# SGI-2022/Latent-Diffusion-Models-for-Shape-SDFs

Measured on AMD Instinct MI355X. Metric: SDF queries/sec on 256^3 grid (+ DDPM sample steps/sec), higher is better.
Workload: dtype bf16; 1 GPU; config4: decode B=64 shapes on a 256^3 grid on 1 rank (the whole grid is the one slab: no gather); batch=64, grid=256, latent_dim=256, decoder=DeepSDF 8x512 skip@4, parallelism=zslab1

## Files before the change

latent-diffusion-models-for-shape-sdfs_amd/csrc/decoder_fs.hip:

```cpp
#include "decoder_common.h"

namespace ldm {
namespace {
using namespace dec;

constexpr int kFsD = 4;

constexpr int kFsStep = 2048;
constexpr int kFsAct = 33 * 4 * 1024;
constexpr int kFsRed = 4 * 4 * 64 * 4;
constexpr int kFsWl = 512 * 4;
#ifndef FS_STAMP
#define FS_STAMP 0
#endif
constexpr int kFsStamp = FS_STAMP ? 128 * 8 : 0;
#ifndef FS_ABL
#define FS_ABL 0
#endif
static_assert(FS_ABL == 0 || FS_STAMP, "ablations are diagnostic builds");
constexpr int kFsLds = kFsAct + kFsRed + kFsWl + kFsStamp;
static_assert(kFsLds <= 160 * 1024, "LDS");

__host__ __device__ constexpr int fs_nparts(int S) { return S == 256 ? 15 : 16; }
__host__ __device__ constexpr int fs_nsteps(int S) { return S == 256 ? 384 : 448; }

template <typename T>
__global__ void fs_aux_pack_kernel(const float* __restrict__ beta, const float* __restrict__ wxyz,
                                   int B, T* __restrict__ aux) {
    const int id = blockIdx.x * blockDim.x + threadIdx.x;
    if (id >= B * 4 * 4 * 2 * 64) return;
    const int lane = id & 63;
    const int i = (id >> 6) & 1;
    const int slot = (id >> 7) & 3;
    const int w = (id >> 9) & 3;
    const int b = id >> 11;
    const int li = slot >> 1;
    const int p = slot & 1;
    float v[8] = {0, 0, 0, 0, 0, 0, 0, 0};
    if (lane < 32) {
        const int f = 128 * w + 64 * p + 32 * i + lane;
        const float* wx = wxyz + ((size_t)li * kHidden + f) * 3;
        const float bb = beta[((size_t)b * 2 + li) * kHidden + f];
        const float hi = Elem<T>::round(bb);
        v[0] = wx[0]; v[1] = wx[1]; v[2] = wx[2];
        v[3] = wx[0]; v[4] = wx[1]; v[5] = wx[2];
        v[6] = hi;    v[7] = bb - hi;
    }
    T* o = aux + (size_t)id * 8;
#pragma unroll
    for (int e = 0; e < 8; ++e) o[e] = (T)v[e];
}

struct FArgs {
    const uint8_t* stream;
    const uint8_t* aux;
    const float* w_last;
    const float* xyz;
    float* out;
    float b_last;
    int npts, tiles_per_shape, n_tiles;
    int N, k0;
    float vs, origin;
    const int32_t* bricks;
    const int32_t* count;
    int nb, nbt;
    GridDiv gd;
};

enum FsEpi { FE_NONE = 0, FE_LATE = 1, FE_EARLY = 2, FE_FIN0 = 3, FE_FIN1 = 4 };

struct FSrc {
    bool shape;
    uint32_t off;
    bool none = false;
};

struct FCtx {
    int lane, wave, h;
    uint32_t voff;
    char* smem;
    __amdgpu_buffer_rsrc_t rw;
    __amdgpu_buffer_rsrc_t ra;
    uint32_t s_beg, s_end;
    uint32_t s_iss;
    uint32_t baux_w;
    uint32_t aux_w;
    uint32_t aux_next;
    u32x4 auxn[2];
    u32x4 ring[kFsD][2];
    u32x4 b[4];
    float part[4];
    float* out;
    int npts, prev_shape, prev_local;
    float b_last;
    unsigned long long* st;
    int st_i;
    bool st_on;
    const int32_t* bricks;
    int N, nb, nbt;
};

__device__ __forceinline__ void stamp(FCtx& c) {
    if (FS_STAMP) {
        if (c.st_on && c.lane == 0 && c.st_i < 128) c.st[c.st_i] = __builtin_readcyclecounter();
        ++c.st_i;
    }
}

__device__ __forceinline__ u32x4 bld(__amdgpu_buffer_rsrc_t r, uint32_t voff, uint32_t soff) {
    return __builtin_bit_cast(u32x4, __builtin_amdgcn_raw_buffer_load_b128(r, voff, soff, 0));
}

__device__ __forceinline__ void load_aux(FCtx& c, FSrc s) {
    if (s.none) return;
    const __amdgpu_buffer_rsrc_t r = s.shape ? c.ra : c.rw;
    c.auxn[0] = bld(r, c.voff, s.off);
    c.auxn[1] = bld(r, c.voff + 1024u, s.off);
}

__device__ __forceinline__ uint32_t opaque(uint32_t v) {
    asm volatile("" : "+v"(v));
    return v;
}

__device__ __forceinline__ int opaque_s(int v) {
    asm volatile("" : "+s"(v));
    return v;
}

__device__ __forceinline__ char* lds_at(const FCtx& c, uint32_t off) {
    return c.smem + (opaque(c.voff) + off);
}
__device__ __forceinline__ u32x4* act_w(const FCtx& c, int late) {
    return reinterpret_cast<u32x4*>(lds_at(c, (uint32_t)(late + 4 * c.wave) * 4096u));
}
__device__ __forceinline__ const f32x4* wl_at(const FCtx& c, int p, int i) {
    const uint32_t h = opaque(c.voff) >> 9;
    return reinterpret_cast<const f32x4*>(
        c.smem + kFsAct + kFsRed + (((c.wave * 2 + p) * 2 + i) * 2) * 64 + h * 64);
}

__device__ __forceinline__ float* red_w(const FCtx& c) {
    return reinterpret_cast<float*>(c.smem + kFsAct + c.wave * 4 * 64 * 4 + (opaque(c.voff) >> 2));
}

__device__ __forceinline__ void fs_bar() {
    if (FS_ABL & 4) return;
    asm volatile("s_waitcnt lgkmcnt(0)\n\ts_barrier" ::: "memory");
}

__device__ __forceinline__ void read_b(FCtx& c, int pos) {
    const u32x4* p = reinterpret_cast<const u32x4*>(lds_at(c, pos * 4096));
#pragma unroll
    for (int n = 0; n < 4; ++n) c.b[n] = p[n * 64];
}

__device__ __forceinline__ void issue(FCtx& c, int r) {
    const uint32_t so = c.s_iss + (uint32_t)(r >> 1) * 2u * kFsStep;
    const uint32_t vo = c.voff + (uint32_t)(r & 1) * kFsStep;
    if (FS_ABL & 1) return;
    c.ring[r][0] = bld(c.rw, vo, so);
    c.ring[r][1] = bld(c.rw, vo + 1024u, so);
}

__device__ __forceinline__ void next_group(FCtx& c) {
    c.s_iss += 4u * kFsStep;
    if (c.s_iss == c.s_end) c.s_iss = c.s_beg;
}

__device__ __forceinline__ float relu_f(float x) {
    return __builtin_bit_cast(float, max(__builtin_bit_cast(int, x), 0));
}

__device__ __forceinline__ float acc_read(float a) {
    asm volatile("" : "+a"(a));
    return a;
}

template <typename T, int EK>
__device__ __forceinline__ void epi_unit(FCtx& c, const f32x16 (&accY)[2][4], int u) {
    const int t = u >> 1, s = u & 1;
    const int i = t >> 2, n = t & 3;
    if (FS_ABL & 2) return;
    if (EK == FE_LATE || EK == FE_EARLY) {
        u32x4 f;
#pragma unroll
        for (int q = 0; q < 4; ++q)
            f[q] = relu2(Elem<T>::pack(accY[i][n][8 * s + 2 * q], accY[i][n][8 * s + 2 * q + 1]));
        u32x4* p = act_w(c, EK == FE_LATE ? 16 : 0);
        p[((2 * i + s) * 4 + n) * 64] = f;
    } else if (EK == FE_FIN0 || EK == FE_FIN1) {
        const f32x4* w = wl_at(c, EK == FE_FIN0 ? 0 : 1, i);
        float part = c.part[n];
#pragma unroll
        for (int q = 2 * s; q < 2 * s + 2; ++q) {
            const f32x4 wv = w[q];
#pragma unroll
            for (int e = 0; e < 4; ++e) {
                const float v = EK == FE_FIN1 ? acc_read(accY[i][n][4 * q + e])
                                              : accY[i][n][4 * q + e];
                part = fmaf(relu_f(v), wv[e], part);
            }
        }
        c.part[n] = part;
    }
}

template <typename T, int EK>
__device__ __forceinline__ void epi_step(FCtx& c, const f32x16 (&accY)[2][4], int k) {
    if (EK == FE_NONE || k == 15) return;
    epi_unit<T, EK>(c, accY, k);
    if (k == 14) epi_unit<T, EK>(c, accY, 15);
    if (EK == FE_FIN1 && k == 14) {
        float* rw = red_w(c);
#pragma unroll
        for (int n = 0; n < 4; ++n) {
            rw[n * 64] = c.part[n];
            c.part[n] = 0.f;
        }
    }
}

__device__ __forceinline__ void fin_store(const FCtx& c, int shape, int local) {
    const int lane = (int)(opaque(c.voff) >> 4);
    if (local < 0 || lane >= 32) return;
    const float* rr = reinterpret_cast<const float*>(
        c.smem + kFsAct + c.wave * 64 * 4 + (opaque(c.voff) >> 2));
    float s = 0.f;
#pragma unroll
    for (int w = 0; w < 4; ++w) s += rr[w * 4 * 64] + rr[w * 4 * 64 + 32];
    const int pt = local * kTilePoints + 32 * c.wave + lane;
    if (pt < c.npts) {
        const __amdgpu_buffer_rsrc_t ro = __builtin_amdgcn_make_buffer_rsrc(
            (void*)(c.out + (size_t)shape * c.npts), (short)0, 0x7ffffff0, 0x00020000);
        __builtin_amdgcn_raw_buffer_store_b32(__builtin_bit_cast(uint32_t, tanhf(s + c.b_last)),
                                              ro, (uint32_t)pt * 4u, 0, 2 );
    }
}

__device__ __forceinline__ int list_at(const int32_t* list, int i) {
    typedef const __attribute__((address_space(4))) int32_t* const_i32;
    return ((const_i32)(uintptr_t)list)[i];
}

__device__ __forceinline__ void brick_origin(int gid, int nb_, int& shape, int& i0, int& j0,
                                             int& k0) {
    const int nb = opaque_s(nb_);
    const int nb2 = nb * nb, nb3 = nb2 * nb;
    shape = gid / nb3;
    const int id = gid - shape * nb3;
    const int bz = id / nb2, r = id - bz * nb2;
    const int by = r / nb;
    i0 = 8 * (r - by * nb);
    j0 = 8 * by;
    k0 = 8 * bz;
}

__device__ __forceinline__ void fin_store_bricks(const FCtx& c, int tile) {
    const int lane = (int)(opaque(c.voff) >> 4);
    if (tile < 0 || lane >= 32) return;
    const float* rr = reinterpret_cast<const float*>(
        c.smem + kFsAct + c.wave * 64 * 4 + (opaque(c.voff) >> 2));
    float s = 0.f;
#pragma unroll
    for (int w = 0; w < 4; ++w) s += rr[w * 4 * 64] + rr[w * 4 * 64 + 32];
    const int gid = list_at(c.bricks, tile >> 2);
    LDM_DASSERT(gid >= 0 && gid < c.nbt);
    int shape, i0, j0, k0;
    brick_origin(gid, c.nb, shape, i0, j0, k0);
    const int idx = 128 * (tile & 3) + 32 * c.wave + lane;
    const int i = i0 + (idx & 7), j = j0 + ((idx >> 3) & 7);
    const int k = k0 + 2 * (tile & 3) + (c.wave >> 1);
    const int N = c.N;
    if ((unsigned)gid < (unsigned)c.nbt && i < N && j < N && k < N) {
        const __amdgpu_buffer_rsrc_t ro = __builtin_amdgcn_make_buffer_rsrc(
            (void*)(c.out + ((size_t)shape * N + k) * N * N), (short)0, 0x7ffffff0, 0x00020000);
        __builtin_amdgcn_raw_buffer_store_b32(__builtin_bit_cast(uint32_t, tanhf(s + c.b_last)),
                                              ro, (uint32_t)(j * N + i) * 4u, 0, 2 );
    }
}

template <int MODE>
__device__ __forceinline__ void fin_store_mode(const FCtx& c) {
    if (MODE == kModeBricks) fin_store_bricks(c, c.prev_local);
    else fin_store(c, c.prev_shape, c.prev_local);
}

__device__ __forceinline__ void valu_slot(int v) {
    if (v == 2) __builtin_amdgcn_sched_group_barrier(0x002, 2, 0);
    else if (v == 4) __builtin_amdgcn_sched_group_barrier(0x002, 4, 0);
}

template <typename T>
__device__ __forceinline__ void mfma_pair(f32x16 (&acc)[2][4], const u32x4& a0, const u32x4& a1,
                                          const u32x4& b, int n) {
    acc[0][n] = Elem<T>::mfma(a0, b, acc[0][n]);
    acc[1][n] = Elem<T>::mfma(a1, b, acc[1][n]);
}

template <typename T, int EK, int K0, int BAR>
__device__ __forceinline__ void group4(FCtx& c, f32x16 (&acc)[2][4], const f32x16 (&accY)[2][4],
                                       int p0) {
    constexpr int BP = 1;
    const char* gbase = lds_at(c, (p0 + 1) * 4096);
#pragma unroll
    for (int r = 0; r < 4; ++r) {
        const u32x4* nb = reinterpret_cast<const u32x4*>(gbase + r * 4096);
        const u32x4 a0 = c.ring[r][0], a1 = c.ring[r][1];
        const int k = K0 + r;
        const int V = (EK == FE_NONE || k == 15) ? 0 : (k == 14 ? 4 : 2);
        if (r == BAR) {
#pragma unroll
            for (int n = 0; n < BP; ++n) mfma_pair<T>(acc, a0, a1, c.b[n], n);
            for (int n = 0; n < BP; ++n) {
                __builtin_amdgcn_sched_group_barrier(0x008, 2, 0);
            }
            __builtin_amdgcn_sched_barrier(0);
            fs_bar();
            __builtin_amdgcn_sched_barrier(0);
#pragma unroll
            for (int n = 0; n < BP; ++n) c.b[n] = nb[n * 64];
#pragma unroll
            for (int n = BP; n < 4; ++n) {
                mfma_pair<T>(acc, a0, a1, c.b[n], n);
                c.b[n] = nb[n * 64];
            }
            issue(c, r);
            epi_step<T, EK>(c, accY, k);
            for (int n = 0; n < BP; ++n) __builtin_amdgcn_sched_group_barrier(0x100, 1, 0);
            for (int n = BP; n < 4; ++n) {
                __builtin_amdgcn_sched_group_barrier(0x008, 1, 0);
                valu_slot(V);
                __builtin_amdgcn_sched_group_barrier(0x008, 1, 0);
                __builtin_amdgcn_sched_group_barrier(0x100, 1, 0);
                valu_slot(V);
            }
        } else {
#pragma unroll
            for (int n = 0; n < 4; ++n) {
                mfma_pair<T>(acc, a0, a1, c.b[n], n);
                c.b[n] = nb[n * 64];
            }
            issue(c, r);
            epi_step<T, EK>(c, accY, k);
#pragma unroll
            for (int n = 0; n < 4; ++n) {
                __builtin_amdgcn_sched_group_barrier(0x008, 1, 0);
                valu_slot(V);
                __builtin_amdgcn_sched_group_barrier(0x008, 1, 0);
                __builtin_amdgcn_sched_group_barrier(0x100, 1, 0);
                valu_slot(V);
            }
        }
        __builtin_amdgcn_sched_group_barrier(0x020, 2, 0);
        __builtin_amdgcn_sched_barrier(0);
    }
    next_group(c);
}

template <typename T, int EK, bool BAR>
__device__ __forceinline__ void steps16e(FCtx& c, f32x16 (&acc)[2][4],
                                         const f32x16 (&accY)[2][4], int p0) {
    group4<T, EK, 0, -1>(c, acc, accY, p0);
    group4<T, EK, 4, -1>(c, acc, accY, p0 + 4);
    group4<T, EK, 8, -1>(c, acc, accY, p0 + 8);
    group4<T, EK, 12, BAR ? 3 : -1>(c, acc, accY, p0 + 12);
}

template <typename T>
__device__ __forceinline__ void steps_plain(FCtx& c, f32x16 (&acc)[2][4],
                                            const f32x16 (&accY)[2][4], int pos0, int j0, int j1) {
#pragma unroll 1
    for (int j = j0; j < j1; j += 4) group4<T, FE_NONE, 0, -1>(c, acc, accY, pos0 + j);
}

template <typename T, int EK, bool E16, int MODE = kModeGrid>
__device__ __forceinline__ void run_part(FCtx& c, f32x16 (&acc)[2][4], const f32x16 (&accY)[2][4],
                                         int nk, bool mid, bool endbar, FSrc naux, int pos0,
                                         bool bar0) {
    const f32x16 zero = {};
    const u32x4 a0 = c.auxn[0], a1 = c.auxn[1];
    if (bar0) {
#pragma unroll
        for (int n = 0; n < 4; ++n) {
            acc[0][n] = Elem<T>::mfma(a0, c.b[n], zero);
            acc[1][n] = Elem<T>::mfma(a1, c.b[n], zero);
        }
        load_aux(c, naux);
        fs_bar();
        read_b(c, pos0);
    } else {
        const u32x4* p = reinterpret_cast<const u32x4*>(lds_at(c, pos0 * 4096));
#pragma unroll
        for (int n = 0; n < 4; ++n) {
            acc[0][n] = Elem<T>::mfma(a0, c.b[n], zero);
            acc[1][n] = Elem<T>::mfma(a1, c.b[n], zero);
            c.b[n] = p[n * 64];
        }
        load_aux(c, naux);
#pragma unroll
        for (int n = 0; n < 4; ++n) {
            __builtin_amdgcn_sched_group_barrier(0x008, 2, 0);
            __builtin_amdgcn_sched_group_barrier(0x100, 1, 0);
        }
        __builtin_amdgcn_sched_group_barrier(0x020, 2, 0);
        __builtin_amdgcn_sched_barrier(0);
    }
    stamp(c);
    if (!E16 && EK != FE_NONE) {
        if (mid || (endbar && nk == 16)) steps16e<T, EK, true>(c, acc, accY, pos0);
        else steps16e<T, EK, false>(c, acc, accY, pos0);
        if (EK == FE_FIN1) {
            stamp(c);
            fin_store_mode<MODE>(c);
        }
        stamp(c);
        if (endbar && nk == 32) {
            steps_plain<T>(c, acc, accY, pos0, 16, 28);
            group4<T, FE_NONE, 0, 3>(c, acc, accY, pos0 + 28);
        } else {
            steps_plain<T>(c, acc, accY, pos0, 16, nk);
        }
    } else if (E16) {
        steps_plain<T>(c, acc, accY, pos0, 0, 12);
        group4<T, FE_NONE, 0, 3>(c, acc, accY, pos0 + 12);
        stamp(c);
        if (endbar) steps16e<T, EK, true>(c, acc, accY, pos0 + 16);
        else steps16e<T, EK, false>(c, acc, accY, pos0 + 16);
    } else {
        steps_plain<T>(c, acc, accY, pos0, 0, nk < 16 ? nk : 16);
        stamp(c);
        steps_plain<T>(c, acc, accY, pos0, 16, nk);
    }
    stamp(c);
}

template <typename T>
__device__ __forceinline__ void acc_to_lds(FCtx& c, const f32x16 (&acc)[2][4]) {
    u32x4* p = act_w(c, 16);
#pragma unroll
    for (int i = 0; i < 2; ++i)
#pragma unroll
        for (int n = 0; n < 4; ++n) {
            u32x4 f0, f1;
            acc_to_frags<T>(acc[i][n], f0, f1);
            p[(2 * i * 4 + n) * 64] = f0;
            p[((2 * i + 1) * 4 + n) * 64] = f1;
        }
}

template <typename T, bool LATE>
__device__ __forceinline__ void layer0_part(FCtx& c, FSrc naux) {
    const u32x4 a[2] = {c.auxn[0], c.auxn[1]};
    u32x4* p = act_w(c, LATE ? 16 : 0);
    f32x16 t[2];
    t[0] = Elem<T>::mfma_v(a[0], c.b[0]);
#pragma unroll
    for (int q = 0; q < 8; ++q) {
        const int i = q & 1, n = q >> 1;
        if (q < 7) t[(q + 1) & 1] = Elem<T>::mfma_v(a[(q + 1) & 1], c.b[(q + 1) >> 1]);
        if (q == 0) {
            asm volatile("s_nop 10" : "+v"(t[0]));
            load_aux(c, naux);
            stamp(c);
        }
        __builtin_amdgcn_sched_barrier(0);
        u32x4 f0, f1;
        acc_to_frags<T>(t[q & 1], f0, f1);
        p[(2 * i * 4 + n) * 64] = f0;
        p[((2 * i + 1) * 4 + n) * 64] = f1;
        __builtin_amdgcn_sched_barrier(0);
    }
    stamp(c);
}

template <typename T, int S, int MODE>
__global__ __launch_bounds__(256, 1) void dec_fs_kernel(FArgs a) {
    __shared__ __attribute__((aligned(16))) char smem[kFsLds];
    FCtx c;
    c.lane = threadIdx.x & 63;
    c.wave = __builtin_amdgcn_readfirstlane(threadIdx.x >> 6);
    c.h = c.lane >> 5;
    c.voff = (uint32_t)c.lane * 16u;
    c.smem = smem;
    c.out = a.out;
    c.npts = a.npts;
    c.b_last = a.b_last;
    c.prev_shape = 0;
    c.prev_local = -1;
    c.st = reinterpret_cast<unsigned long long*>(smem + kFsAct + kFsRed + kFsWl);
    c.st_i = 0;
    c.st_on = false;
    float* wl = reinterpret_cast<float*>(smem + kFsAct + kFsRed);

    for (int i = threadIdx.x; i < 512; i += 256) wl[i] = a.w_last[i];
    __syncthreads();
    const int n_tiles = MODE == kModeBricks ? 4 * min(max(a.count[0], 0), a.nbt) : a.n_tiles;
    if (MODE == kModeBricks) {
        c.bricks = a.bricks;
        c.N = a.N;
        c.nb = a.nb;
        c.nbt = a.nbt;
    }
    if ((int)blockIdx.x >= n_tiles) return;

    constexpr int NST = fs_nsteps(S);
    constexpr int NP = fs_nparts(S);
    constexpr uint32_t kFlags = 0x00020000u;
    c.rw = __builtin_amdgcn_make_buffer_rsrc((void*)a.stream, (short)0, 0x7ffffff0, kFlags);
    c.ra = __builtin_amdgcn_make_buffer_rsrc((void*)a.aux, (short)0, 0x7ffffff0, kFlags);
    c.s_beg = (uint32_t)c.wave * NST * kFsStep;
    c.s_end = c.s_beg + NST * kFsStep;
    c.s_iss = c.s_beg;
    c.baux_w = (uint32_t)(4 * NST + c.wave * NP) * kFsStep;
    auto brick_of = [&](int tile) -> int {
        return min(max(list_at(a.bricks, tile >> 2), 0), a.nbt - 1);
    };
    auto shape_aux = [&](int tile) -> uint32_t {
        if (MODE == kModeBricks) {
            const int nb = opaque_s(a.nb);
            return ((uint32_t)(brick_of(tile) / (nb * nb * nb)) * 4u + (uint32_t)c.wave) * 4u *
                   kFsStep;
        }
        return ((uint32_t)(tile / a.tiles_per_shape) * 4u + (uint32_t)c.wave) * 4u * kFsStep;
    };
    auto bias = [&](int pi) -> FSrc { return FSrc{false, c.baux_w + (uint32_t)pi * kFsStep}; };
    auto shp = [&](int slot) -> FSrc { return FSrc{true, c.aux_w + (uint32_t)slot * kFsStep}; };
    c.aux_w = shape_aux(blockIdx.x);
#pragma unroll
    for (int r = 0; r < kFsD; ++r) issue(c, r);
    next_group(c);

    f32x16 accA[2][4], accB[2][4];
#pragma unroll
    for (int i = 0; i < 2; ++i)
#pragma unroll
        for (int n = 0; n < 4; ++n) accB[i][n] = f32x16{};
#pragma unroll
    for (int n = 0; n < 4; ++n) c.part[n] = 0.f;
#pragma unroll 1
    for (int tile = blockIdx.x; tile < n_tiles; tile += gridDim.x) {
        int shape, local, bi0 = 0, bj0 = 0, bk0 = 0;
        if (MODE == kModeBricks) {
            brick_origin(brick_of(tile), a.nb, shape, bi0, bj0, bk0);
            local = tile;
        } else {
            shape = tile / a.tiles_per_shape;
            local = tile - shape * a.tiles_per_shape;
        }
        {
            const int nt = tile + (int)gridDim.x;
            c.aux_next = nt < n_tiles ? shape_aux(nt) : c.aux_w;
        }
        c.st_on = FS_STAMP && c.wave == 0 && tile == (int)blockIdx.x + (int)gridDim.x;
        c.st_i = 0;
        stamp(c);
        load_aux(c, shp(0));
        const uint32_t lv = opaque(c.voff);
        const bool hi = lv >= 512u;
        const uint32_t p0 = (uint32_t)local * kTilePoints;
        uint32_t ti = 0, tj = 0, tk = 0;
        if (MODE == kModeGrid) {
            grid_first(p0, (uint32_t)a.N, a.gd, ti, tj, tk);
            tk += (uint32_t)a.k0;
        }
        const float* row = nullptr;
        if (MODE == kModePoints) {
            row = a.xyz + (size_t)shape * a.npts * 3;
            asm volatile("" : "+s"(row));
        }
#pragma unroll
        for (int n = 0; n < 4; ++n) {
            int pt = local * kTilePoints + 32 * n + (int)((lv >> 4) & 31u);
            if (pt >= a.npts) pt = a.npts - 1;
            float x, y, z;
            if (MODE == kModeBricks) {
                const int idx = 128 * (tile & 3) + 32 * n + (int)((lv >> 4) & 31u);
                const int m = a.N - 1;
                x = grid_axis(min(bi0 + (idx & 7), m), a.vs, a.origin);
                y = grid_axis(min(bj0 + ((idx >> 3) & 7), m), a.vs, a.origin);
                z = grid_axis(min(bk0 + (idx >> 6), m), a.vs, a.origin);
            } else if (MODE == kModePoints) {
                const float* qq = row + (size_t)pt * 3;
                x = qq[0];
                y = qq[1];
                z = qq[2];
            } else {
                const uint32_t off =
                    grid_tail_off(p0, 32u * n + ((lv >> 4) & 31u), (uint32_t)a.npts);
                uint32_t vi, vj, vk;
                grid_voxel(ti, tj, tk, off, (uint32_t)a.N, a.gd.m, vi, vj, vk);
                x = grid_axis((int)vi, a.vs, a.origin);
                y = grid_axis((int)vj, a.vs, a.origin);
                z = grid_axis((int)vk, a.vs, a.origin);
            }
            const float xh = Elem<T>::round(x), yh = Elem<T>::round(y), zh = Elem<T>::round(z);
            u32x4 f;
            f[0] = hi ? 0u : Elem<T>::pack(xh, yh);
            f[1] = hi ? 0u : Elem<T>::pack(zh, x - xh);
            f[2] = hi ? 0u : Elem<T>::pack(y - yh, z - zh);
            f[3] = hi ? 0u : Elem<T>::pack(1.f, 1.f);
            reinterpret_cast<u32x4*>(lds_at(c, 32u * 4096u))[n * 64] = f;
        }
        read_b(c, 32);

        layer0_part<T, false>(c, shp(1));
        layer0_part<T, true>(c, bias(2));

        int pi = 2;
        run_part<T, FE_FIN1, false, MODE>(c, accA, accB, 32, true, false, bias(pi + 1), 0, true);
        run_part<T, FE_EARLY, true>(c, accB, accA, 32, true, true, bias(pi + 2), 0, false);
        pi += 2;
        constexpr int L2P = S == 256 ? 3 : 4;
#pragma unroll 1
        for (int l = 2; l < L2P; ++l, pi += 2) {
            const FSrc nx = (S == 512 && l == 3) ? shp(2) : bias(pi + 2);
            run_part<T, FE_LATE, false>(c, accA, accB, 32, true, false, bias(pi + 1), 0, false);
            run_part<T, FE_EARLY, true>(c, accB, accA, 32, true, true, nx, 0, false);
        }
        if (S == 256) {
            run_part<T, FE_LATE, false>(c, accA, accB, 32, true, false, shp(2), 0, false);
            fs_bar();
            acc_to_lds<T>(c, accA);
            stamp(c);
            run_part<T, FE_NONE, false>(c, accA, accB, 16, false, false, shp(3), 16, true);
            run_part<T, FE_EARLY, false>(c, accB, accA, 16, false, true, bias(pi + 3), 16,
                                             false);
            pi += 3;
        } else {
            run_part<T, FE_LATE, false>(c, accA, accB, 32, true, false, shp(3), 0, false);
            run_part<T, FE_EARLY, true>(c, accB, accA, 32, true, true, bias(pi + 2), 0, false);
            pi += 2;
        }
#pragma unroll 1
        for (int l = 5; l < 7; ++l, pi += 2) {
            run_part<T, FE_LATE, false>(c, accA, accB, 32, true, false, bias(pi + 1), 0, false);
            run_part<T, FE_EARLY, true>(c, accB, accA, 32, true, true, bias(pi + 2), 0, false);
        }
        run_part<T, FE_LATE, false>(c, accA, accB, 32, true, false, bias(pi + 1), 0, false);
        run_part<T, FE_FIN0, false>(c, accB, accA, 32, false, true, FSrc{true, 0, true}, 0,
                                        false);
        c.prev_shape = shape;
        c.prev_local = local;
        c.aux_w = c.aux_next;
    }
#pragma unroll
    for (int u = 0; u < 16; ++u) epi_unit<T, FE_FIN1>(c, accB, u);
    {
        float* rw = red_w(c);
#pragma unroll
        for (int n = 0; n < 4; ++n) rw[n * 64] = c.part[n];
    }
    fs_bar();
    fin_store_mode<MODE>(c);
    asm volatile("s_waitcnt vmcnt(0)" ::: "memory");
    if (FS_STAMP && c.wave == 0) {
        __builtin_amdgcn_s_waitcnt(0);
        for (int k = c.lane; k < 128; k += 64)
            reinterpret_cast<unsigned long long*>(a.out)[(size_t)blockIdx.x * 128 + k] = c.st[k];
    }
}

template <typename T, int S>
void launch_fs(const FArgs& a, bool points, hipStream_t s, int grid) {
    if (points)
        hipLaunchKernelGGL((dec_fs_kernel<T, S, kModePoints>), dim3(grid), dim3(256), 0, s, a);
    else
        hipLaunchKernelGGL((dec_fs_kernel<T, S, kModeGrid>), dim3(grid), dim3(256), 0, s, a);
}

template <typename T, int S>
void launch_fs_bricks(const FArgs& a, hipStream_t s, int grid) {
    hipLaunchKernelGGL((dec_fs_kernel<T, S, kModeBricks>), dim3(grid), dim3(256), 0, s, a);
}

}

size_t decoder_fs_aux_bytes(int B) { return (size_t)B * 4 * 4 * kFsStep; }

int decoder_fs_n_stages(int skip_width) { return fs_nsteps(skip_width == 253 ? 256 : 512); }

int decoder_fs_fwd(const ldm_decoder_t* w, const float* beta, const float* xyz, int B, int npts,
                   int N, int k0, float vs, float origin, float* out, void* ws, size_t ws_bytes,
                   hipStream_t s, int num_cus, const int32_t* bricks, const int32_t* count,
                   int n_bricks) {
    const int S = w->skip_width == 253 ? 256 : 512;
    LDM_REQUIRE(w->n_stages == fs_nsteps(S), LDM_EINVAL, "split layout: n_stages %d != %d",
                w->n_stages, fs_nsteps(S));
    LDM_REQUIRE(ws != nullptr && ws_bytes >= decoder_fs_aux_bytes(B) && LDM_ALIGNED(ws, 16),
                LDM_ENOSPC, "workspace too small: need %zu bytes, got %zu",
                decoder_fs_aux_bytes(B), ws_bytes);
    LDM_REQUIRE((size_t)B * 4 * 4 * kFsStep < 0x7ffffff0u, LDM_EINVAL,
                "split layout: %d shapes exceed the aux buffer range", B);
    {
        const int n = B * 4 * 4 * 2 * 64;
        if (w->dtype == LDM_BF16)
            hipLaunchKernelGGL(fs_aux_pack_kernel<__bf16>, dim3((n + 255) / 256), dim3(256), 0, s,
                               beta, w->wxyz, B, (__bf16*)ws);
        else
            hipLaunchKernelGGL(fs_aux_pack_kernel<_Float16>, dim3((n + 255) / 256), dim3(256), 0,
                               s, beta, w->wxyz, B, (_Float16*)ws);
        if (int e = launch_status("fs_aux_pack")) return e;
    }
    FArgs a;
    a.stream = (const uint8_t*)w->weights;
    a.aux = (const uint8_t*)ws;
    a.w_last = w->w_last;
    a.xyz = xyz;
    a.out = out;
    a.b_last = w->b_last;
    a.npts = npts;
    a.tiles_per_shape = (npts + kTilePoints - 1) / kTilePoints;
    a.n_tiles = B * a.tiles_per_shape;
    a.bricks = bricks;
    a.count = count;
    a.nb = (N + 7) / 8;
    a.nbt = n_bricks;
    const int mode = bricks ? kModeBricks : xyz ? kModePoints : kModeGrid;
    if (mode == kModeBricks) a.n_tiles = 4 * n_bricks;
    a.N = N;
    a.k0 = k0;
    a.vs = vs;
    a.origin = origin;
    a.gd = mode == kModeGrid ? grid_div(N) : GridDiv{0, 0, 0};
    const int grid = a.n_tiles < num_cus ? a.n_tiles : num_cus;
    if (mode != kModeBricks) {
        const bool points = mode == kModePoints;
        if (w->dtype == LDM_BF16) {
            if (S == 256) launch_fs<__bf16, 256>(a, points, s, grid);
            else launch_fs<__bf16, 512>(a, points, s, grid);
        } else {
            if (S == 256) launch_fs<_Float16, 256>(a, points, s, grid);
            else launch_fs<_Float16, 512>(a, points, s, grid);
        }
    } else if (w->dtype == LDM_BF16) {
        if (S == 256) launch_fs_bricks<__bf16, 256>(a, s, grid);
        else launch_fs_bricks<__bf16, 512>(a, s, grid);
    } else {
        if (S == 256) launch_fs_bricks<_Float16, 256>(a, s, grid);
        else launch_fs_bricks<_Float16, 512>(a, s, grid);
    }
    return launch_status("ldm_decoder_fwd(split)");
}

}
```

Measured before the change: 475.2 million queries/s.

## Pin epilogue accumulator reads in AGPRs and split E16 conversion into convert/write phases

Adds a PIN flag so most epilogues read accumulators through an AGPR asm constraint. This keeps the compiler from copying whole accumulator tiles into VGPRs early. For S=256 the E16 path now converts half of the layer's accumulators into a 16-entry register buffer while MFMAs run, then writes them to LDS in a separate group. The other layers keep the original late/early epilogue interleave. The aim is lower register pressure and better overlap of the epilogue with MFMA, at the cost of extra live registers (ef[16]) and a more intricate schedule.

```diff
diff --git a/latent-diffusion-models-for-shape-sdfs_amd/csrc/decoder_fs.hip b/latent-diffusion-models-for-shape-sdfs_amd/csrc/decoder_fs.hip
--- a/latent-diffusion-models-for-shape-sdfs_amd/csrc/decoder_fs.hip
+++ b/latent-diffusion-models-for-shape-sdfs_amd/csrc/decoder_fs.hip
@@ -67,7 +67,8 @@
     GridDiv gd;
 };
 
-enum FsEpi { FE_NONE = 0, FE_LATE = 1, FE_EARLY = 2, FE_FIN0 = 3, FE_FIN1 = 4 };
+enum FsEpi { FE_NONE = 0, FE_LATE = 1, FE_EARLY = 2, FE_FIN0 = 3, FE_FIN1 = 4, FE_CVT = 5,
+             FE_WR = 6, FE_PIN = 8 };
 
 struct FSrc {
     bool shape;
@@ -90,6 +91,7 @@
     u32x4 ring[kFsD][2];
     u32x4 b[4];
     float part[4];
+    u32x4 ef[16];
     float* out;
     int npts, prev_shape, prev_local;
     float b_last;
@@ -177,18 +179,22 @@
     return a;
 }
 
-template <typename T, int EK>
-__device__ __forceinline__ void epi_unit(FCtx& c, const f32x16 (&accY)[2][4], int u) {
+template <typename T, int EKP>
+__device__ __forceinline__ void epi_unit(FCtx& c, const f32x16 (&accY)[2][4], int u,
+                                         u32x4* wbase) {
+    constexpr int EK = EKP & 7;
+    constexpr bool PIN = (EKP & FE_PIN) != 0 || EK == FE_FIN1;
     const int t = u >> 1, s = u & 1;
     const int i = t >> 2, n = t & 3;
     if (FS_ABL & 2) return;
     if (EK == FE_LATE || EK == FE_EARLY) {
         u32x4 f;
 #pragma unroll
-        for (int q = 0; q < 4; ++q)
-            f[q] = relu2(Elem<T>::pack(accY[i][n][8 * s + 2 * q], accY[i][n][8 * s + 2 * q + 1]));
-        u32x4* p = act_w(c, EK == FE_LATE ? 16 : 0);
-        p[((2 * i + s) * 4 + n) * 64] = f;
+        for (int q = 0; q < 4; ++q) {
+            const float lo = accY[i][n][8 * s + 2 * q], hi = accY[i][n][8 * s + 2 * q + 1];
+            f[q] = relu2(PIN ? Elem<T>::pack(acc_read(lo), acc_read(hi)) : Elem<T>::pack(lo, hi));
+        }
+        wbase[((2 * i + s) * 4 + n) * 64] = f;
     } else if (EK == FE_FIN0 || EK == FE_FIN1) {
         const f32x4* w = wl_at(c, EK == FE_FIN0 ? 0 : 1, i);
         float part = c.part[n];
@@ -197,8 +203,7 @@
             const f32x4 wv = w[q];
 #pragma unroll
             for (int e = 0; e < 4; ++e) {
-                const float v = EK == FE_FIN1 ? acc_read(accY[i][n][4 * q + e])
-                                              : accY[i][n][4 * q + e];
+                const float v = PIN ? acc_read(accY[i][n][4 * q + e]) : accY[i][n][4 * q + e];
                 part = fmaf(relu_f(v), wv[e], part);
             }
         }
@@ -206,11 +211,40 @@
     }
 }
 
-template <typename T, int EK>
-__device__ __forceinline__ void epi_step(FCtx& c, const f32x16 (&accY)[2][4], int k) {
+template <typename T, int EKP>
+__device__ __forceinline__ void epi_step(FCtx& c, const f32x16 (&accY)[2][4], int k,
+                                         u32x4* wbase) {
+    constexpr int EK = EKP & 7;
     if (EK == FE_NONE || k == 15) return;
-    epi_unit<T, EK>(c, accY, k);
-    if (k == 14) epi_unit<T, EK>(c, accY, 15);
+    if (EK == FE_CVT) {
+        if ((FS_ABL & 2) || k >= 8) return;
+        u32x4 f0, f1;
+#pragma unroll
+        for (int q = 0; q < 4; ++q) {
+            const f32x16& a = accY[k >> 2][k & 3];
+            f0[q] = relu2(Elem<T>::pack(acc_read(a[2 * q]), acc_read(a[2 * q + 1])));
+            f1[q] = relu2(Elem<T>::pack(acc_read(a[8 + 2 * q]), acc_read(a[8 + 2 * q + 1])));
+        }
+        c.ef[2 * k] = f0;
+        c.ef[2 * k + 1] = f1;
+        return;
+    }
+    if (EK == FE_WR) {
+        if ((FS_ABL & 2) || k >= 4) return;
+#pragma unroll
+        for (int t = 2 * k; t < 2 * k + 2; ++t) {
+            const int i = t >> 2, n = t & 3;
+            wbase[(2 * i * 4 + n) * 64] = c.ef[2 * t];
+            wbase[((2 * i + 1) * 4 + n) * 64] = c.ef[2 * t + 1];
+        }
+        return;
+    }
+    epi_unit<T, EKP>(c, accY, k, wbase);
+    if (k == 14) epi_unit<T, EKP>(c, accY, 15, wbase);
+    if (EK == FE_FIN0 && k == 14) {
+#pragma unroll
+        for (int n = 0; n < 4; ++n) asm volatile("" : "+v"(c.part[n]));
+    }
     if (EK == FE_FIN1 && k == 14) {
         float* rw = red_w(c);
 #pragma unroll
@@ -298,17 +332,22 @@
     acc[1][n] = Elem<T>::mfma(a1, b, acc[1][n]);
 }
 
-template <typename T, int EK, int K0, int BAR>
+template <typename T, int EKP, int K0, int BAR>
 __device__ __forceinline__ void group4(FCtx& c, f32x16 (&acc)[2][4], const f32x16 (&accY)[2][4],
                                        int p0) {
+    constexpr int EK = EKP & 7;
     constexpr int BP = 1;
+    u32x4* wbase = nullptr;
+    if (EK == FE_LATE) wbase = act_w(c, 16);
+    if (EK == FE_EARLY || EK == FE_WR) wbase = act_w(c, 0);
     const char* gbase = lds_at(c, (p0 + 1) * 4096);
 #pragma unroll
     for (int r = 0; r < 4; ++r) {
         const u32x4* nb = reinterpret_cast<const u32x4*>(gbase + r * 4096);
         const u32x4 a0 = c.ring[r][0], a1 = c.ring[r][1];
         const int k = K0 + r;
-        const int V = (EK == FE_NONE || k == 15) ? 0 : (k == 14 ? 4 : 2);
+        const int V = (EK == FE_NONE || EK == FE_WR || k == 15) ? 0
+                      : (k == 14 || EK == FE_CVT) ? 4 : 2;
         if (r == BAR) {
 #pragma unroll
             for (int n = 0; n < BP; ++n) mfma_pair<T>(acc, a0, a1, c.b[n], n);
@@ -326,7 +365,7 @@
                 c.b[n] = nb[n * 64];
             }
             issue(c, r);
-            epi_step<T, EK>(c, accY, k);
+            epi_step<T, EKP>(c, accY, k, wbase);
             for (int n = 0; n < BP; ++n) __builtin_amdgcn_sched_group_barrier(0x100, 1, 0);
             for (int n = BP; n < 4; ++n) {
                 __builtin_amdgcn_sched_group_barrier(0x008, 1, 0);
@@ -342,7 +381,7 @@
                 c.b[n] = nb[n * 64];
             }
             issue(c, r);
-            epi_step<T, EK>(c, accY, k);
+            epi_step<T, EKP>(c, accY, k, wbase);
 #pragma unroll
             for (int n = 0; n < 4; ++n) {
                 __builtin_amdgcn_sched_group_barrier(0x008, 1, 0);
@@ -374,10 +413,11 @@
     for (int j = j0; j < j1; j += 4) group4<T, FE_NONE, 0, -1>(c, acc, accY, pos0 + j);
 }
 
-template <typename T, int EK, bool E16, int MODE = kModeGrid>
+template <typename T, int EKP, bool E16, int MODE = kModeGrid>
 __device__ __forceinline__ void run_part(FCtx& c, f32x16 (&acc)[2][4], const f32x16 (&accY)[2][4],
                                          int nk, bool mid, bool endbar, FSrc naux, int pos0,
                                          bool bar0) {
+    constexpr int EK = EKP & 7;
     const f32x16 zero = {};
     const u32x4 a0 = c.auxn[0], a1 = c.auxn[1];
     if (bar0) {
@@ -406,10 +446,16 @@
         __builtin_amdgcn_sched_group_barrier(0x020, 2, 0);
         __builtin_amdgcn_sched_barrier(0);
     }
+    if (EK == FE_NONE) {
+#pragma unroll
+        for (int i = 0; i < 2; ++i)
+#pragma unroll
+            for (int n = 0; n < 4; ++n) asm volatile("" ::"a"(accY[i][n]));
+    }
     stamp(c);
     if (!E16 && EK != FE_NONE) {
-        if (mid || (endbar && nk == 16)) steps16e<T, EK, true>(c, acc, accY, pos0);
-        else steps16e<T, EK, false>(c, acc, accY, pos0);
+        if (mid || (endbar && nk == 16)) steps16e<T, EKP, true>(c, acc, accY, pos0);
+        else steps16e<T, EKP, false>(c, acc, accY, pos0);
         if (EK == FE_FIN1) {
             stamp(c);
             fin_store_mode<MODE>(c);
@@ -421,12 +467,21 @@
         } else {
             steps_plain<T>(c, acc, accY, pos0, 16, nk);
         }
-    } else if (E16) {
+    } else if (E16 && (EKP & FE_PIN)) {
         steps_plain<T>(c, acc, accY, pos0, 0, 12);
         group4<T, FE_NONE, 0, 3>(c, acc, accY, pos0 + 12);
         stamp(c);
-        if (endbar) steps16e<T, EK, true>(c, acc, accY, pos0 + 16);
-        else steps16e<T, EK, false>(c, acc, accY, pos0 + 16);
+        if (endbar) steps16e<T, EKP, true>(c, acc, accY, pos0 + 16);
+        else steps16e<T, EKP, false>(c, acc, accY, pos0 + 16);
+    } else if (E16) {
+        static_assert(!E16 || EK == FE_EARLY, "E16 parts convert part 0 of their own layer");
+        steps_plain<T>(c, acc, accY, pos0, 0, 8);
+        group4<T, FE_CVT, 0, -1>(c, acc, accY, pos0 + 8);
+        group4<T, FE_CVT, 4, 3>(c, acc, accY, pos0 + 12);
+        stamp(c);
+        group4<T, FE_WR, 0, -1>(c, acc, accY, pos0 + 16);
+        steps_plain<T>(c, acc, accY, pos0, 20, 28);
+        group4<T, FE_NONE, 0, 3>(c, acc, accY, pos0 + 28);
     } else {
         steps_plain<T>(c, acc, accY, pos0, 0, nk < 16 ? nk : 16);
         stamp(c);
@@ -607,6 +662,7 @@
         layer0_part<T, false>(c, shp(1));
         layer0_part<T, true>(c, bias(2));
 
+        constexpr int kPinW = S == 512 ? FE_PIN : 0;
         int pi = 2;
         run_part<T, FE_FIN1, false, MODE>(c, accA, accB, 32, true, false, bias(pi + 1), 0, true);
         run_part<T, FE_EARLY, true>(c, accB, accA, 32, true, true, bias(pi + 2), 0, false);
@@ -615,37 +671,44 @@
 #pragma unroll 1
         for (int l = 2; l < L2P; ++l, pi += 2) {
             const FSrc nx = (S == 512 && l == 3) ? shp(2) : bias(pi + 2);
-            run_part<T, FE_LATE, false>(c, accA, accB, 32, true, false, bias(pi + 1), 0, false);
-            run_part<T, FE_EARLY, true>(c, accB, accA, 32, true, true, nx, 0, false);
+            run_part<T, FE_LATE | kPinW, false>(c, accA, accB, 32, true, false, bias(pi + 1), 0,
+                                                false);
+            run_part<T, FE_EARLY | FE_PIN, true>(c, accB, accA, 32, true, true, nx, 0, false);
         }
         if (S == 256) {
-            run_part<T, FE_LATE, false>(c, accA, accB, 32, true, false, shp(2), 0, false);
+            run_part<T, FE_LATE | kPinW, false>(c, accA, accB, 32, true, false, shp(2), 0,
+                                                false);
             fs_bar();
             acc_to_lds<T>(c, accA);
             stamp(c);
             run_part<T, FE_NONE, false>(c, accA, accB, 16, false, false, shp(3), 16, true);
-            run_part<T, FE_EARLY, false>(c, accB, accA, 16, false, true, bias(pi + 3), 16,
-                                             false);
+            run_part<T, FE_EARLY | FE_PIN, false>(c, accB, accA, 16, false, true, bias(pi + 3),
+                                                  16, false);
             pi += 3;
         } else {
-            run_part<T, FE_LATE, false>(c, accA, accB, 32, true, false, shp(3), 0, false);
-            run_part<T, FE_EARLY, true>(c, accB, accA, 32, true, true, bias(pi + 2), 0, false);
+            run_part<T, FE_LATE | kPinW, false>(c, accA, accB, 32, true, false, shp(3), 0,
+                                                false);
+            run_part<T, FE_EARLY | FE_PIN, true>(c, accB, accA, 32, true, true, bias(pi + 2), 0,
+                                                 false);
             pi += 2;
         }
 #pragma unroll 1
         for (int l = 5; l < 7; ++l, pi += 2) {
-            run_part<T, FE_LATE, false>(c, accA, accB, 32, true, false, bias(pi + 1), 0, false);
-            run_part<T, FE_EARLY, true>(c, accB, accA, 32, true, true, bias(pi + 2), 0, false);
-        }
-        run_part<T, FE_LATE, false>(c, accA, accB, 32, true, false, bias(pi + 1), 0, false);
-        run_part<T, FE_FIN0, false>(c, accB, accA, 32, false, true, FSrc{true, 0, true}, 0,
-                                        false);
+            run_part<T, FE_LATE | FE_PIN, false>(c, accA, accB, 32, true, false, bias(pi + 1), 0,
+                                                 false);
+            run_part<T, FE_EARLY | FE_PIN, true>(c, accB, accA, 32, true, true, bias(pi + 2), 0,
+                                                 false);
+        }
+        run_part<T, FE_LATE | FE_PIN, false>(c, accA, accB, 32, true, false, bias(pi + 1), 0,
+                                             false);
+        run_part<T, FE_FIN0 | FE_PIN, false>(c, accB, accA, 32, false, true, FSrc{true, 0, true},
+                                             0, false);
         c.prev_shape = shape;
         c.prev_local = local;
         c.aux_w = c.aux_next;
     }
 #pragma unroll
-    for (int u = 0; u < 16; ++u) epi_unit<T, FE_FIN1>(c, accB, u);
+    for (int u = 0; u < 16; ++u) epi_unit<T, FE_FIN1>(c, accB, u, nullptr);
     {
         float* rw = red_w(c);
 #pragma unroll
```

Measured after the change: 480.0 million queries/s, median of 6. +1.0%, better.
